# sail-sg/finetune-fair-diffusion

Measured on AMD Instinct MI355X. Metric: training-images/sec (SD-v1.5 512^2, 20-step DPM-Solver++ unroll, fairness-finetune step), higher is better.
Workload: dtype f16

## Files before the change

finetune_fair_diffusion_amd/csrc/gemm.hip:

```cpp
#include "gemm_device.h"

template <int BM, int BN, bool CONV>
__global__ __launch_bounds__(256) void gemm_glds_kernel(fd_gemm_desc p, int ntm, int ntn) {
    FD_WG_TRACE(1);
    constexpr int TM = BM / 32, TN = BN / 32;
    constexpr int AI = BM / 64, BI = BN / 64;
    constexpr int EPI_HALFS = 4 * (BM / 2) * (BN / 2 + 4);
    constexpr int OPS_HALFS = 2 * (BM + BN) * 32;
    __shared__ __attribute__((aligned(16))) f16 smem[OPS_HALFS > EPI_HALFS ? OPS_HALFS : EPI_HALFS];
    f16* As = smem;
    f16* Bs = smem + 2 * BM * 32;
    const f16* zp = fd_zero_page;
    asm volatile("" : "+s"(zp));

    const int tid = threadIdx.x, lane = tid & 63, wave = tid >> 6;
    const int l15 = lane & 15, lg = lane >> 4;
    const int wm = wave >> 1, wn = wave & 1;

    const int tile = xcd_remap(blockIdx.x, ntm * ntn);
    const int m0 = (tile / ntn) * BM, n0 = (tile % ntn) * BN;
    const int z = blockIdx.y;

    const f16* A = (const f16*)p.A + (int64_t)z * p.sA;
    const f16* B = (const f16*)p.B + (int64_t)z * p.sB;
// ... 278 lines not shown
            const bool kok = kk < Kseg;
#pragma unroll
            for (int i = 0; i < AI; ++i) {
                const int g = wave + i * NW;
                if (g < NA && (part & 1)) {
                    const int m = m0 + g * 8 + lrow;
                    const f16* src = (kok && m < p.M) ? Ap + (int64_t)m * la + kk : zp;
                    glds16(src, As + (buf * BM + g * 8) * 64);
                }
            }
#pragma unroll
            for (int i = 0; i < BI; ++i) {
                const int g = wave + i * NW;
                if (g < NB && (part & 2)) {
                    const int n = n0 + g * 8 + lrow;
                    const f16* src = (kok && n < p.N) ? Bp + (int64_t)n * lb + kk : zp;
                    glds16(src, Bs + (buf * BN + g * 8) * 64);
                }
            }
        }
    };

    f32x4 acc[TM][TN];
#pragma unroll
    for (int i = 0; i < TM; ++i)
#pragma unroll
        for (int j = 0; j < TN; ++j) acc[i][j] = (f32x4){0.f, 0.f, 0.f, 0.f};

    const int frow = l15 * 64;
    const int fsw = l15 & 7;
    const uint32_t lds0 = (uint32_t)(uintptr_t)(__attribute__((address_space(3))) void*)smem;
    constexpr bool PINNED = NW == 8;
#ifndef FD_PD
#define FD_PD 2
#endif

    const int nsplit = gridDim.y;
    const int kbeg = (int)((int64_t)nk * blockIdx.y / nsplit), kend = (int)((int64_t)nk * (blockIdx.y + 1) / nsplit);
    issue(kbeg, 0, 3);
    for (int kt = kbeg; kt < (FD_DBG_GE(p, 4) ? kbeg : kend); ++kt) {
        const int buf = (kt - kbeg) & 1;
        asm volatile("s_waitcnt vmcnt(0)" ::: "memory");
        __syncthreads();
        if (kt + 1 < kend && !FD_DBG_IS(p, 1)) issue(kt + 1, buf ^ 1, 3);
        if (FD_DBG_IS(p, 2)) continue;
        if constexpr (PINNED) {
            const uint32_t a_base = lds0 + (uint32_t)((buf * BM + wm * WTM) * 64 + frow) * 2;
            const uint32_t b_base = lds0 + (uint32_t)((2 * BM + buf * BN + wn * WTN) * 64 + frow) * 2;
#pragma unroll
            for (int ks = 0; ks < 2; ++ks) {
                const uint32_t slot = (uint32_t)(((ks * 4 + lg) ^ fsw) * 16);
                mma_k32<TM, TN, FD_PD>(acc, a_base + slot, b_base + slot);
            }
        } else {
            const f16* Ab = As + (buf * BM + wm * WTM) * 64 + frow;
            const f16* Bb = Bs + (buf * BN + wn * WTN) * 64 + frow;
#pragma unroll
            for (int ks = 0; ks < 2; ++ks) {
                const int slot = ((ks * 4 + lg) ^ fsw) * 8;
                if (TN <= TM) {
                    f16x8 bf[TN];
#pragma unroll
                    for (int j = 0; j < TN; ++j) bf[j] = *(const f16x8*)(Bb + j * 16 * 64 + slot);
                    f16x8 a0 = *(const f16x8*)(Ab + slot);
                    f16x8 a1 = *(const f16x8*)(Ab + (TM > 1 ? 1 : 0) * 16 * 64 + slot);
#pragma unroll
                    for (int i = 0; i < TM; ++i) {
                        f16x8 a2 = a1;
                        if (i + 2 < TM) a2 = *(const f16x8*)(Ab + (i + 2) * 16 * 64 + slot);
#pragma unroll
                        for (int j = 0; j < TN; ++j) acc[i][j] = FD_MFMA_16x16x32(bf[j], a0, acc[i][j]);
                        __builtin_amdgcn_sched_group_barrier(0x100, 1, 0);
                        __builtin_amdgcn_sched_group_barrier(0x008, TN, 0);
                        a0 = a1;
                        a1 = a2;
                    }
                } else {
                    f16x8 af[TM];
#pragma unroll
                    for (int i = 0; i < TM; ++i) af[i] = *(const f16x8*)(Ab + i * 16 * 64 + slot);
                    f16x8 b0 = *(const f16x8*)(Bb + slot);
                    f16x8 b1 = *(const f16x8*)(Bb + (TN > 1 ? 1 : 0) * 16 * 64 + slot);
#pragma unroll
                    for (int j = 0; j < TN; ++j) {
                        f16x8 b2 = b1;
                        if (j + 2 < TN) b2 = *(const f16x8*)(Bb + (j + 2) * 16 * 64 + slot);
#pragma unroll
                        for (int i = 0; i < TM; ++i) acc[i][j] = FD_MFMA_16x16x32(b0, af[i], acc[i][j]);
                        __builtin_amdgcn_sched_group_barrier(0x100, 1, 0);
                        __builtin_amdgcn_sched_group_barrier(0x008, TM, 0);
                        b0 = b1;
                        b1 = b2;
                    }
                }
            }
        }
    }

    if (nsplit > 1) {
        float* ws = (float*)p.workspace + (int64_t)blockIdx.y * p.M * p.N;
#pragma unroll
        for (int i = 0; i < TM; ++i) {
            const int m = m0 + wm * WTM + i * 16 + l15;
            if (m >= p.M) continue;
#pragma unroll
            for (int j = 0; j < TN; ++j) {
                const int n = n0 + wn * WTN + j * 16 + lg * 4;
                if (n < p.N) *(f32x4*)(ws + (int64_t)m * p.N + n) = acc[i][j];
            }
        }
        return;
    }
    const bool lds_epi = FD_GEMM_LDS_EPILOGUE_OK(p);
    if (FD_DBG_IS(p, 3)) {
        if (acc[0][0][0] == 12345.678f) ((f16*)p.C)[0] = (f16)1.f;
    } else if (p.act == FD_ACT_GEGLU) {
        constexpr int LDS_HALFS = 2 * (BM + BN) * 64;
        constexpr int TMC = (NW * WTM * (WTN + 4) <= LDS_HALFS) ? TM : TM / 2;
        __syncthreads();
        gemm_epilogue_geglu_lds<TM, TN, TMC>(p, acc, smem + wave * (TMC * 16) * (WTN + 4), m0 + wm * WTM, n0 + wn * WTN, lane);
    } else if (lds_epi) {
        constexpr int LDS_HALFS = 2 * (BM + BN) * 64;
        constexpr int TMC = (NW * WTM * (WTN + 4) <= LDS_HALFS) ? TM : TM / 2;
        static_assert(NW * TMC * 16 * (WTN + 4) <= LDS_HALFS, "epilogue staging does not fit");
        __syncthreads();
        gemm_epilogue_lds<TM, TN, TMC, WSTATS>(p, acc, smem + wave * (TMC * 16) * (WTN + 4), m0 + wm * WTM, n0 + wn * WTN, lane, 0, 0, up_phase);
    } else {
        gemm_epilogue<TM, TN>(p, acc, m0 + wm * WTM, n0 + wn * WTN, l15, lg, 0, 0, up_phase);
    }
}

__global__ void splitk_reduce_kernel(fd_gemm_desc p, int nsplit) {
    FD_WG_TRACE(3);
    const int64_t n4 = (int64_t)p.M * p.N / 4;
    const float* ws = (const float*)p.workspace;
    const f16* R = (const f16*)p.residual;
    const f16* RB = (const f16*)p.rowbias;
    for (int64_t i = blockIdx.x * (int64_t)blockDim.x + threadIdx.x; i < n4; i += (int64_t)gridDim.x * blockDim.x) {
        const int64_t e = i * 4;
        const int m = (int)(e / p.N), n = (int)(e - (int64_t)m * p.N);
        f32x4 a = *(const f32x4*)(ws + e);
        for (int s = 1; s < nsplit; ++s) a += *(const f32x4*)(ws + (int64_t)s * p.M * p.N + e);
        const int rbrow = RB ? m / p.rows_per_batch : 0;
        float v[4];
        const float al = n < p.colscale_cols ? p.alpha * p.colscale : p.alpha;
#pragma unroll
        for (int r = 0; r < 4; ++r) {
            float x = a[r] * al;
            if (p.bias) x += p.bias[n + r];
            if (RB) x += (float)RB[(int64_t)rbrow * p.ld_rowbias + n + r];
            x = apply_act(x, p.act);
            if (R) x += (float)R[(int64_t)m * p.ldr + n + r];
            v[r] = x;
        }
        if (p.out_dtype == FD_OUT_F32) *(f32x4*)((float*)p.C + (int64_t)m * p.ldc + n) = (f32x4){v[0], v[1], v[2], v[3]};
        else *(f16x4*)((f16*)p.C + (int64_t)m * p.ldc + n) = (f16x4){(f16)v[0], (f16)v[1], (f16)v[2], (f16)v[3]};
    }
}

static int launch_splitk_reduce(const fd_gemm_desc& d, hipStream_t s, int nsplit) {
    int64_t blocks = ((int64_t)d.M * d.N / 4 + 255) / 256;
    if (blocks > 2048) blocks = 2048;
    hipLaunchKernelGGL(splitk_reduce_kernel, dim3((unsigned)blocks), dim3(256), 0, s, d, nsplit);
    return fd_check_launch("fd_gemm(split-K reduce)");
}

template <auto KERNEL, int NTHREADS, size_t LDS>
static void launch_big_cv(const fd_gemm_desc& d, hipStream_t s, dim3 grid, int ntm, int ntn, int gn) {
    fd_allow_lds<KERNEL>(LDS);
    hipLaunchKernelGGL(KERNEL, grid, dim3(NTHREADS), LDS, s, d, ntm, ntn, gn);
}

template <int BM, int BN, int WGM, int WGN>
static int launch_big(const fd_gemm_desc& d, hipStream_t s, int nsplit, int cv) {
    const int ntm = (d.M + BM - 1) / BM, ntn = (d.N + BN - 1) / BN;
    constexpr size_t lds = (size_t)2 * (BM + BN) * 64 * sizeof(f16);
    constexpr int nt = WGM * WGN * 64;
    static const long l2_budget = bench_env("FD_GEMM_L2_KB") ? atol(bench_env("FD_GEMM_L2_KB")) * 1024 : GEMM_L2_BUDGET;
    const int gn = gemm_band_ntiles(l2_budget, BN, ((long)d.K + d.K2) / nsplit, ntn);
    const int nph = (d.conv && (d.conv_mode == FD_CONV_UP2P || d.conv_mode == FD_CONV_UP2PI)) ? 4 : 1;
    const dim3 grid(ntm * ntn * nph, nsplit);
    if (cv == 0) launch_big_cv<gemm_big_kernel<BM, BN, WGM, WGN, 0>, nt, lds>(d, s, grid, ntm, ntn, gn);
    else if (cv == 1) launch_big_cv<gemm_big_kernel<BM, BN, WGM, WGN, 1>, nt, lds>(d, s, grid, ntm, ntn, gn);
    else if (cv == 2) launch_big_cv<gemm_big_kernel<BM, BN, WGM, WGN, 2>, nt, lds>(d, s, grid, ntm, ntn, gn);
    else if constexpr (BN / WGN == 80) {
        if (cv == 6) launch_big_cv<gemm_big_kernel<BM, BN, WGM, WGN, 6>, nt, lds>(d, s, grid, ntm, ntn, gn);
        else if (cv == 3) launch_big_cv<gemm_big_kernel<BM, BN, WGM, WGN, 3>, nt, lds>(d, s, grid, ntm, ntn, gn);
        else launch_big_cv<gemm_big_kernel<BM, BN, WGM, WGN, 4>, nt, lds>(d, s, grid, ntm, ntn, gn);
    }
    if (nsplit > 1) return launch_splitk_reduce(d, s, nsplit);
    return fd_check_launch(cv >= 3 ? "fd_gemm(big, statistics epilogue)" : "fd_gemm(big)");
}


template <int NT, int KS, int RT>
__global__ __launch_bounds__(KS * 64) void gemm_skinny_kernel(fd_gemm_desc p) {
    FD_WG_TRACE(4);
    __shared__ float red[KS > 1 ? (KS - 1) * RT * NT * 256 : 1];
    const int lane = threadIdx.x & 63, wave = threadIdx.x >> 6;
    const int l15 = lane & 15, lg = lane >> 4;
    const f16* A[RT];
    bool mok[RT];
#pragma unroll
    for (int r = 0; r < RT; ++r) {
        const int m = (blockIdx.x * RT + r) * 16 + l15;
        mok[r] = m < p.M;
        A[r] = (const f16*)p.A + (int64_t)(mok[r] ? m : 0) * p.lda + lg * 8;
    }
    const f16* B = (const f16*)p.B + lg * 8;
    f32x4 acc[RT][NT];
#pragma unroll
    for (int r = 0; r < RT; ++r)
#pragma unroll
        for (int j = 0; j < NT; ++j) acc[r][j] = (f32x4){0.f, 0.f, 0.f, 0.f};
    const int nks = p.K >> 5;
    const int per = (nks + KS - 1) / KS;
    const int kbeg = wave * per, kend = min(nks, kbeg + per);
    constexpr int CH = 10 / RT;
    for (int k0 = kbeg; k0 < kend; k0 += CH) {
        f16x8 af[RT][CH];
#pragma unroll
        for (int c = 0; c < CH; ++c)
#pragma unroll
            for (int r = 0; r < RT; ++r) {
                af[r][c] = (f16x8){0, 0, 0, 0, 0, 0, 0, 0};
                if (k0 + c < kend && mok[r]) af[r][c] = *(const f16x8*)(A[r] + (int64_t)(k0 + c) * 32);
            }
#pragma unroll
        for (int c = 0; c < CH; ++c) {
            if (k0 + c < kend) {
#pragma unroll
                for (int j = 0; j < NT; ++j) {
                    const int n = j * 16 + l15;
                    f16x8 bf = (f16x8){0, 0, 0, 0, 0, 0, 0, 0};
                    if (n < p.N) bf = *(const f16x8*)(B + (int64_t)n * p.ldb + (int64_t)(k0 + c) * 32);
#pragma unroll
                    for (int r = 0; r < RT; ++r) acc[r][j] = FD_MFMA_16x16x32(bf, af[r][c], acc[r][j]);
                }
            }
        }
    }
    if (KS > 1) {
        if (wave > 0) {
#pragma unroll
            for (int r = 0; r < RT; ++r)
#pragma unroll
                for (int j = 0; j < NT; ++j) *(f32x4*)(red + ((((wave - 1) * RT + r) * NT + j) * 64 + lane) * 4) = acc[r][j];
        }
        __syncthreads();
        if (wave > 0) return;
#pragma unroll
        for (int w = 1; w < KS; ++w)
#pragma unroll
            for (int r = 0; r < RT; ++r)
#pragma unroll
                for (int j = 0; j < NT; ++j) acc[r][j] += *(const f32x4*)(red + ((((w - 1) * RT + r) * NT + j) * 64 + lane) * 4);
    }
#pragma unroll
    for (int r = 0; r < RT; ++r) {
        if (!mok[r]) continue;
        f16* C = (f16*)p.C + (int64_t)((blockIdx.x * RT + r) * 16 + l15) * p.ldc;
#pragma unroll
        for (int j = 0; j < NT; ++j) {
            const int n = j * 16 + lg * 4;
            if (n < p.N) *(f16x4*)(C + n) = (f16x4){(f16)acc[r][j][0], (f16)acc[r][j][1], (f16)acc[r][j][2], (f16)acc[r][j][3]};
        }
    }
}

static bool skinny_ok(const fd_gemm_desc& d) {
    static const bool off = bench_env("FD_GEMM_NOSKINNY") != nullptr;
    if (d.N > 16 && d.M >= 32768) return false;
    return !off && !d.conv && d.batch <= 1 && d.K2 == 0 && d.colscale_cols == 0 && d.N <= 64 && (d.N & 3) == 0 && (d.K & 31) == 0 && d.M >= 1024 && !d.bias && !d.rowbias &&
           !d.residual && d.act == FD_ACT_NONE && d.alpha == 1.f && d.out_dtype == FD_OUT_F16 && (d.ldc & 3) == 0;
}

template <int NT, int RT>
static int launch_skinny_rt(const fd_gemm_desc& d, hipStream_t s) {
    const int blocks = (d.M + 16 * RT - 1) / (16 * RT);
    const int ks = d.K >= 1280 ? 4 : d.K >= 640 ? 2 : 1;
    if (ks == 4) hipLaunchKernelGGL((gemm_skinny_kernel<NT, 4, RT>), dim3(blocks), dim3(256), 0, s, d);
    else if (ks == 2) hipLaunchKernelGGL((gemm_skinny_kernel<NT, 2, RT>), dim3(blocks), dim3(128), 0, s, d);
    else hipLaunchKernelGGL((gemm_skinny_kernel<NT, 1, RT>), dim3(blocks), dim3(64), 0, s, d);
    return fd_check_launch("fd_gemm(skinny)");
}

template <int NT>
static int launch_skinny(const fd_gemm_desc& d, hipStream_t s) {
    static const int rt = bench_env("FD_GEMM_SKINNY_RT") ? atoi(bench_env("FD_GEMM_SKINNY_RT")) : 0;
    const bool two = rt == 2;
    return two ? launch_skinny_rt<NT, 2>(d, s) : launch_skinny_rt<NT, 1>(d, s);
}

template <int BM, int BN>
static int launch(const fd_gemm_desc& d, hipStream_t s) {
    const int ntm = (d.M + BM - 1) / BM, ntn = (d.N + BN - 1) / BN;
    dim3 grid(ntm * ntn, d.batch > 0 ? d.batch : 1);
    if (d.conv) hipLaunchKernelGGL((gemm_glds_kernel<BM, BN, true>), grid, dim3(256), 0, s, d, ntm, ntn);
    else hipLaunchKernelGGL((gemm_glds_kernel<BM, BN, false>), grid, dim3(256), 0, s, d, ntm, ntn);
    return fd_check_launch("fd_gemm");
}

bool fd_gemm_pp_eligible(const fd_gemm_desc& d);
int fd_gemm_launch_pp(const fd_gemm_desc& d, hipStream_t s, bool prio, int bm, int nsplit);
bool fd_conv_halo_takes(const fd_gemm_desc& d, int bm, int nsplit);
#ifndef FD_GEMM_PP_DEFAULT
#define FD_GEMM_PP_DEFAULT (1 | 4 | 8 | 32)
#endif
static int pp_mode() {
#ifdef FD_BENCH_HOOKS
    const char* e = getenv("FD_GEMM_PP");
    return e ? atoi(e) : FD_GEMM_PP_DEFAULT;
#else
    return FD_GEMM_PP_DEFAULT;
#endif
}
static int pp_takes(const fd_gemm_desc& d, int sel) {
    const int t = sel % 1000000, split = sel / 1000000, m = pp_mode();
    if (!m || !fd_gemm_pp_eligible(d)) return 0;
    if (t == 256320 && split == 0) {
        if (d.conv) return (m & 1) ? 256 : 0;
        if ((m & 2) || ((m & 32) && d.K + d.K2 <= 384 && d.N >= 2560)) return 256;
        return 0;
    }
    if (t == 128320 && (split == 0 || (m & 64))) return (m & (d.conv ? 8 : 16)) ? 128 : 0;
    return 0;
}

static int gemm_tile(const fd_gemm_desc& d);
extern "C" int fd_gemm_tile(const fd_gemm_desc* dp) {
    FD_REQUIRE_DESC(dp, fd_gemm_desc, "fd_gemm_tile");
    return gemm_tile(*dp);
}
static int gemm_tile(const fd_gemm_desc& d) {
    const long nb = d.batch > 1 ? d.batch : 1;
    static const bool nobig = bench_env("FD_GEMM_NOBIG") != nullptr;
    static const int force = bench_env("FD_GEMM_FORCE") ? atoi(bench_env("FD_GEMM_FORCE")) : 0;
    if (skinny_ok(d)) return 16000 + (d.N + 15) / 16 * 16;
    if (force && nb == 1 && !d.conv) return force;
    static const int bigk = bench_env("FD_GEMM_BIGK") ? atoi(bench_env("FD_GEMM_BIGK")) : 320;
    if (!nobig && nb == 1 && (d.conv ? (d.Cin & 63) == 0 : (d.K + d.K2) >= bigk)) {
        const long phs = (d.conv && (d.conv_mode == FD_CONV_UP2P || d.conv_mode == FD_CONV_UP2PI)) ? 4 : 1;
        const long m256 = phs * ((d.M + 255) / 256), m128 = phs * ((d.M + 127) / 128);
        static const long t256 = bench_env("FD_GEMM_T256") ? atol(bench_env("FD_GEMM_T256")) : 100;
        static const long t128 = bench_env("FD_GEMM_T128") ? atol(bench_env("FD_GEMM_T128")) : 80;
        static const long maxsplit = bench_env("FD_GEMM_MAXSPLIT") ? atol(bench_env("FD_GEMM_MAXSPLIT")) : 8;
        static const long tc256 = bench_env("FD_CONV_T256") ? atol(bench_env("FD_CONV_T256")) : 0;
        if (d.N % 320 == 0) {
            if (m256 * (d.N / 320) >= ((tc256 && d.conv && d.conv_mode == FD_CONV_NORMAL) ? tc256 : t256)) return 256320;
            if (m128 * (d.N / 320) >= t128) return 128320;
        }
        const bool can_split = d.workspace && (d.N & 3) == 0 && (d.ldc & 3) == 0 && d.act != FD_ACT_GEGLU && phs == 1;
        const long nk = (d.K + 63) / 64 + (d.K2 + 63) / 64;
        auto split_for = [&](long blocks, int tilecode) -> int {
            long split = blocks > 0 ? 256 / blocks : 1;
            if (split > maxsplit) split = maxsplit;
            while (split > 1 && (nk / split < 8 || (int64_t)split * d.M * d.N * 4 > d.workspace_bytes)) --split;
            return split > 1 ? (int)(split * 1000000 + tilecode) : 0;
        };
        if (can_split && nk >= 64 && d.N % 320 == 0 && m128 * (d.N / 320) >= 32) {
            const int c = split_for(m128 * (d.N / 320), 128320);
            if (c) return c;
        }
        static const long t160 = bench_env("FD_GEMM_T160") ? atol(bench_env("FD_GEMM_T160")) : 160;
        if (d.N % 160 == 0 && m128 * (d.N / 160) >= t160) return 128160;
        static const bool no256 = bench_env("FD_GEMM_NO256256") != nullptr;
        static const long tvae = bench_env("FD_GEMM_TVAE") ? atol(bench_env("FD_GEMM_TVAE")) : 200;
        if (!no256 && d.N % 256 == 0 && m256 * (d.N / 256) >= tvae) return 256256;
        static const bool no512 = bench_env("FD_GEMM_NO512128") != nullptr;
        if (!no512 && d.N == 128 && ((d.M + 511) / 512) >= 400) return 512128;
        if (d.N % 128 == 0 && m256 * (d.N / 128) >= tvae) return 256128;
        if (can_split && d.N % 160 == 0) {
            const int c = split_for(m128 * (d.N / 160), 128160);
            if (c) return c;
        }
    }
    const long t128 = (long)((d.M + 127) / 128) * ((d.N + 127) / 128) * nb;
    const bool n64 = (d.N % 128) != 0 && (d.N % 128) <= 64;
    if (t128 >= 512 && !n64) return 128128;
    const long t12864 = (long)((d.M + 127) / 128) * ((d.N + 63) / 64) * nb;
    if (t12864 >= 512) return 128064;
    return 64064;
}

enum { GK_SKINNY, GK_GLDS, GK_BIG, GK_PP };
struct GemmPlan {
    int kind, bm, bn, wgm, wgn, nsplit, cv;
    bool stats_ok;
    int big_cv(bool st) const { return st ? (cv == 2 ? 6 : cv + 3) : cv; }
};
static fd_gemm_desc normalise_k2(fd_gemm_desc d) {
    if (d.K2 <= 0 || !d.A2) d.K2 = 0;
    return d;
}
static GemmPlan gemm_plan(const fd_gemm_desc& d ) {
    GemmPlan g = {};
    const int sel = gemm_tile(d), t = sel % 1000000;
    static const bool w16 = bench_env("FD_GEMM_W8") == nullptr;
    g.nsplit = sel >= 1000000 ? sel / 1000000 : 1;
    g.bm = t / 1000; g.bn = t % 1000;
    g.cv = d.conv ? (d.conv_mode >= FD_CONV_UP2P ? 2 : 1) : 0;
    if (const int bm = pp_takes(d, sel)) { g.kind = GK_PP; g.bm = bm; g.bn = 320; g.wgm = 2; g.wgn = 4; }
    else if (g.nsplit > 1) { g.kind = GK_BIG; g.wgm = 4; g.wgn = t == 128320 ? 4 : 2; }
    else switch (t) {
        case 256320: g.kind = GK_BIG; g.wgm = (w16 && !d.conv) ? 4 : 2; g.wgn = 4; break;
        case 128320: g.kind = GK_BIG; g.wgm = w16 ? 4 : 2; g.wgn = 4; break;
        case 128160: g.kind = GK_BIG; g.wgm = 4; g.wgn = 2; break;
        case 256256: g.kind = GK_BIG; g.wgm = 2; g.wgn = 4; break;
        case 512128: g.kind = GK_BIG; g.wgm = 8; g.wgn = 2; break;
        case 256128: g.kind = GK_BIG; g.wgm = 4; g.wgn = 2; break;
        default: g.kind = g.bm == 16 ? GK_SKINNY : GK_GLDS; break;
    }
    g.stats_ok = (g.kind == GK_PP || (g.kind == GK_BIG && g.bn / g.wgn == 80)) && g.nsplit == 1 && FD_GEMM_LDS_EPILOGUE_OK(d) && d.act != FD_ACT_GEGLU &&
                 d.batch <= 1 && (d.N % 80) == 0 && (g.cv < 2 || (d.conv_mode == FD_CONV_UP2PI && (d.M & 31) == 0));
    return g;
}

extern "C" int fd_gemm_kernel_name(const fd_gemm_desc* dp, char* buf, int n) {
    FD_REQUIRE_DESC(dp, fd_gemm_desc, "fd_gemm_kernel_name");
    const fd_gemm_desc d = normalise_k2(*dp);
    const GemmPlan g = gemm_plan(d);
    const bool st = d.gn_stats && g.stats_ok;
    switch (g.kind) {
        case GK_PP:
            if (fd_conv_halo_takes(d, g.bm, g.nsplit)) snprintf(buf, n, "conv_halo_kernel<%d, %d, %d, true>", g.bm, d.W, st ? 3 : 1);
            else snprintf(buf, n, "gemm_pp_kernel<%d, %d, %s>", g.bm, (d.conv ? 1 : 0) + (st ? 2 : 0), (pp_mode() & 4) ? "true" : "false");
            break;
        case GK_BIG: snprintf(buf, n, "gemm_big_kernel<%d, %d, %d, %d, %d>", g.bm, g.bn, g.wgm, g.wgn, g.big_cv(st)); break;
        case GK_SKINNY: snprintf(buf, n, "gemm_skinny_kernel<%d, %d, 1>", g.bn / 16, d.K >= 1280 ? 4 : d.K >= 640 ? 2 : 1); break;
        default: snprintf(buf, n, "gemm_glds_kernel<%d, %d, %s>", g.bm, g.bn, d.conv ? "true" : "false"); break;
    }
    return g.nsplit > 1 ? g.nsplit : 0;
}

extern "C" int fd_gemm_stats_rows(const fd_gemm_desc* dp) {
    FD_REQUIRE_DESC(dp, fd_gemm_desc, "fd_gemm_stats_rows");
    return gemm_plan(normalise_k2(*dp)).stats_ok ? 32 : 0;
}

extern "C" int fd_gemm(const fd_gemm_desc* dp, void* stream) {
    FD_REQUIRE_DESC(dp, fd_gemm_desc, "fd_gemm");
    fd_gemm_desc d = *dp;
#ifdef FD_BENCH_HOOKS
    static const char* dbg = bench_env("FD_GEMM_DBG");
    if (dbg && d.batch <= 1) d.batch = -atoi(dbg);
#endif
    FD_REQUIRE(d.A && d.B && d.C, "fd_gemm: null operand");
    FD_REQUIRE(d.M > 0 && d.N > 0 && d.K > 0, "fd_gemm: bad shape M=%d N=%d K=%d", d.M, d.N, d.K);
    FD_REQUIRE((d.K & 7) == 0 && (d.lda & 7) == 0 && (d.ldb & 7) == 0, "fd_gemm: K, lda, ldb must be multiples of 8");
    if (d.K2 > 0) {
        FD_REQUIRE(!d.conv, "fd_gemm: second K-slab not supported with conv gather");
        FD_REQUIRE(d.A2 && d.B2 && (d.K2 & 7) == 0 && (d.lda2 & 7) == 0 && (d.ldb2 & 7) == 0, "fd_gemm: bad second slab");
        FD_REQUIRE(d.batch <= 1, "fd_gemm: second slab is not batched");
    }
    d = normalise_k2(d);
    if (d.conv) {
        const bool up_fwd = d.conv_mode == FD_CONV_UP2P || d.conv_mode == FD_CONV_UP2PI;
        const int ntap = up_fwd ? 4 : d.conv_mode == FD_CONV_UP2P_BWD ? 16 : 9;
        FD_REQUIRE((d.Cin & 31) == 0 && d.K == ntap * d.Cin, "fd_gemm(conv): Cin must be a multiple of 32 and K == taps*Cin");
        if (up_fwd) FD_REQUIRE(!d.residual && !d.rowbias, "fd_gemm(conv up2 phases): bias-only epilogue");
        if (d.conv_mode == FD_CONV_UP2PI) FD_REQUIRE(d.out_dtype == FD_OUT_F16, "fd_gemm(conv up2 phases, interleaved result): fp16 output");
        FD_REQUIRE(d.M == d.Bn * d.Ho * d.Wo, "fd_gemm(conv): M != B*Ho*Wo");
        FD_REQUIRE(d.batch <= 1, "fd_gemm(conv): not batched");
        FD_REQUIRE((int64_t)d.Bn * d.H * d.W * d.lda < (1LL << 31), "fd_gemm(conv): input larger than 2^31 elements");
    }
    if (d.rowbias) FD_REQUIRE(d.rows_per_batch > 0, "fd_gemm: rows_per_batch");
    FD_REQUIRE(d.colscale_cols >= 0 && (d.colscale_cols & 3) == 0 && (d.colscale_cols == 0 || (d.act != FD_ACT_GEGLU && d.batch <= 1)),
               "fd_gemm: colscale_cols=%d must be a multiple of 4 (not with GEGLU / batched launches)", d.colscale_cols);
    if (d.act == FD_ACT_GEGLU)
        FD_REQUIRE(!d.conv && d.batch <= 1 && d.out_dtype == FD_OUT_F16 && !d.rowbias && d.alpha == 1.f && (d.N & 15) == 0 &&
                       (d.ldc & 7) == 0 && d.K2 == 0 && (!d.residual || (d.ldr & 7) == 0),
                   "fd_gemm(GEGLU): needs a plain fp16 GEMM with N %% 16 == 0 and ldc, ldr %% 8 == 0");
    hipStream_t s = (hipStream_t)stream;
    const GemmPlan g = gemm_plan(d);
    if (d.gn_stats) FD_REQUIRE(g.stats_ok, "fd_gemm: gn_stats set but the kernel for M=%d N=%d K=%d has no statistics epilogue (ask fd_gemm_stats_rows first)",
                               d.M, d.N, d.K);
    if (d.conv && d.conv_mode >= FD_CONV_UP2P)
        FD_REQUIRE(g.kind == GK_BIG, "fd_gemm(conv up2 phases): shape not taken by the big-tile kernels (Cin %% 64, enough tiles); use FD_CONV_UP2");
    switch (g.kind) {
        case GK_PP: {
            const int rc = fd_gemm_launch_pp(d, s, (pp_mode() & 4) != 0, g.bm, g.nsplit);
            if (rc != 0 || g.nsplit == 1) return rc;
            return launch_splitk_reduce(d, s, g.nsplit);
        }
        case GK_SKINNY:
            switch (g.bn) {
                case 16: return launch_skinny<1>(d, s);
                case 32: return launch_skinny<2>(d, s);
                case 48: return launch_skinny<3>(d, s);
                default: return launch_skinny<4>(d, s);
            }
        case GK_BIG: {
            const int cv = g.big_cv(d.gn_stats != nullptr);
            switch (g.bm * 1000 + g.bn) {
                case 256320: return g.wgm == 4 ? launch_big<256, 320, 4, 4>(d, s, g.nsplit, cv) : launch_big<256, 320, 2, 4>(d, s, g.nsplit, cv);
                case 128320: return g.wgm == 4 ? launch_big<128, 320, 4, 4>(d, s, g.nsplit, cv) : launch_big<128, 320, 2, 4>(d, s, g.nsplit, cv);
                case 128160: return launch_big<128, 160, 4, 2>(d, s, g.nsplit, cv);
                case 256256: return launch_big<256, 256, 2, 4>(d, s, g.nsplit, cv);
                case 512128: return launch_big<512, 128, 8, 2>(d, s, g.nsplit, cv);
                default: return launch_big<256, 128, 4, 2>(d, s, g.nsplit, cv);
            }
        }
        default:
            if (g.bm == 128 && g.bn == 128) return launch<128, 128>(d, s);
            if (g.bm == 128 && g.bn == 64) return launch<128, 64>(d, s);
            return launch<64, 64>(d, s);
    }
}

FD_WGT_SETTER(gemm)
```

finetune_fair_diffusion_amd/csrc/gemm_pp.hip:

```cpp
#include "gemm_pp_device.h"

constexpr uint32_t PP_OOR = 0xFFFFFFF0u;
template <int BM, int CV, bool PRIO>
__global__ __launch_bounds__(512) void gemm_pp_kernel(fd_gemm_desc p, int ntm, int ntn, int gn) {
    FD_WG_TRACE(5);
    constexpr int CONV = CV & 1;
    constexpr bool WSTATS = CV >= 2;
    constexpr int WTM = BM / 2, WTN = 80, TM = WTM / 16, TN = 5;
    constexpr int NGA = BM / 16, NAW = NGA / PP_NW;
    constexpr int STAGE = pp_stage<BM>();
    extern __shared__ __attribute__((aligned(16))) f16 smem[];
    const f16* zp = fd_zero_page;
    asm volatile("" : "+s"(zp));

    const int tid = threadIdx.x, lane = tid & 63;
    const int wave = __builtin_amdgcn_readfirstlane(tid >> 6);
    const int l15 = lane & 15, lg = lane >> 4;
    const int wm = wave >> 2, wn = wave & 3;
    const bool lead = wave < 4;

    int tile = xcd_remap(blockIdx.x, gridDim.x);
    int mt, nt;
    if (gn >= ntn) {
        mt = tile / ntn;
        nt = tile - mt * ntn;
    } else {
        const int per = ntm * gn, nbands = (ntn + gn - 1) / gn;
        const int band = min(tile / per, nbands - 1);
        const int r = tile - band * per;
        const int w = band == nbands - 1 ? ntn - band * gn : gn;
        mt = r / w;
        nt = band * gn + (r - mt * w);
    }
    const int m0 = mt * BM, n0 = nt * PP_BN;

    const f16* A = (const f16*)p.A;
    const f16* B = (const f16*)p.B;
    const int nk1 = (p.K + 31) >> 5, nk2 = (p.K2 + 31) >> 5, nkt = nk1 + nk2;
    const int nsplit = gridDim.y;
    const int kbeg = (int)((int64_t)nkt * blockIdx.y / nsplit), kend = (int)((int64_t)nkt * (blockIdx.y + 1) / nsplit);
    const int nk = kend - kbeg;

    const int lrow = lane >> 2;
    const int kchunk = ((lane & 3) ^ swz_g(lane >> 4)) * 8;
    int a_off[NAW], a_mask[NAW];
#pragma unroll
    for (int i = 0; i < NAW; ++i) {
        const int m = m0 + (wave + 8 * i) * 16 + lrow;
        const bool valid = m < p.M;
        if (CONV) {
            const int hw = p.Ho * p.Wo;
            const int mm = valid ? m : 0;
            const int b = mm / hw;
            const int r = mm - b * hw;
            const int oy = r / p.Wo;
            const int ox = r - oy * p.Wo;
            int mask = 0;
#pragma unroll
            for (int t = 0; t < 9; ++t) {
                const int iy = oy + t / 3 - 1, ix = ox + t % 3 - 1;
                if (valid && iy >= 0 && iy < p.H && ix >= 0 && ix < p.W) mask |= 1 << t;
            }
            a_off[i] = (int)(((int64_t)(b * p.H + oy) * p.W + ox) * p.lda) + kchunk;
            a_mask[i] = mask;
        } else {
            a_off[i] = valid ? m : -1;
            a_mask[i] = 0;
        }
    }
    int b_row[3];
#pragma unroll
    for (int i = 0; i < 3; ++i) {
        const int n = n0 + (wave + 8 * i) * 16 + lrow;
        b_row[i] = (n < p.N && (wave + 8 * i) < PP_NGB) ? n : -1;
    }
    f16* const dump = smem + PP_NST * STAGE + wave * PP_GROUP;
#if __HIP_DEVICE_COMPILE__
    __amdgpu_buffer_rsrc_t rA, rB, rA2, rB2;
    uint32_t a_vo[NAW], a_vo2[NAW], b_vo[3], b_vo2[3];
    if (!CONV) {
        auto rsrc = [](const void* base, int64_t rows, int64_t ld, int k) {
            const int64_t bytes = base ? ((rows - 1) * ld + k) * 2 : 0;
            return __builtin_amdgcn_make_buffer_rsrc((void*)base, 0, (int)(uint32_t)bytes, 0x00020000);
        };
        rA = rsrc(p.A, p.M, p.lda, p.K); rB = rsrc(p.B, p.N, p.ldb, p.K);
        rA2 = rsrc(p.K2 ? p.A2 : nullptr, p.M, p.lda2, p.K2); rB2 = rsrc(p.K2 ? p.B2 : nullptr, p.N, p.ldb2, p.K2);
#pragma unroll
        for (int i = 0; i < NAW; ++i) {
            a_vo[i] = a_off[i] >= 0 ? (uint32_t)(a_off[i] * (int)p.lda + kchunk) * 2 : PP_OOR;
            a_vo2[i] = a_off[i] >= 0 ? (uint32_t)(a_off[i] * (int)p.lda2 + kchunk) * 2 : PP_OOR;
        }
#pragma unroll
        for (int i = 0; i < 3; ++i) {
            b_vo[i] = b_row[i] >= 0 ? (uint32_t)(b_row[i] * (int)p.ldb + kchunk) * 2 : PP_OOR;
            b_vo2[i] = b_row[i] >= 0 ? (uint32_t)(b_row[i] * (int)p.ldb2 + kchunk) * 2 : PP_OOR;
        }
    }
#endif

    auto issue = [&](int j, auto nl_c) {
        constexpr int NL = decltype(nl_c)::value;
        if (j >= nk || (FD_DBG_IS(p, 1) && j >= 3)) {
#pragma unroll
            for (int i = 0; i < NL; ++i) glds16(zp, dump);
            return;
        }
        const int kt = kbeg + j;
        f16* st = smem + (j & 3) * STAGE;
        if (CONV) {
            const int cc = kt / 9;
            const int tap = kt - cc * 9;
            const int c0 = cc << 5;
            const int ky = tap / 3, kx = tap - ky * 3;
            const int toff = ((ky - 1) * p.W + (kx - 1)) * (int)p.lda + c0;
#pragma unroll
            for (int i = 0; i < NAW; ++i) {
                const f16* src = ((a_mask[i] >> tap) & 1) ? A + (int64_t)(a_off[i] + toff) : zp;
                glds16(src, st + (wave + 8 * i) * PP_GROUP);
            }
            const int kk = tap * p.Cin + c0 + kchunk;
#pragma unroll
            for (int i = 0; i < NL - NAW; ++i) {
                const f16* src = b_row[i] >= 0 ? B + (int64_t)b_row[i] * p.ldb + kk : zp;
                glds16(src, st + (NGA + wave + 8 * i) * PP_GROUP);
            }
        } else {
#if __HIP_DEVICE_COMPILE__
            const bool seg2 = kt >= nk1;
            const int k0 = (seg2 ? kt - nk1 : kt) * 32;
            const int rem = (seg2 ? p.K2 : p.K) - k0;
            const bool kok = kchunk < rem;
            const uint32_t so = (uint32_t)k0 * 2;
            if (!seg2) {
#pragma unroll
                for (int i = 0; i < NAW; ++i)
                    __builtin_amdgcn_raw_ptr_buffer_load_lds(rA, (__attribute__((address_space(3))) void*)(st + (wave + 8 * i) * PP_GROUP), 16, kok ? a_vo[i] : PP_OOR, so, 0, 0);
#pragma unroll
                for (int i = 0; i < NL - NAW; ++i)
                    __builtin_amdgcn_raw_ptr_buffer_load_lds(rB, (__attribute__((address_space(3))) void*)(st + (NGA + wave + 8 * i) * PP_GROUP), 16, kok ? b_vo[i] : PP_OOR, so, 0, 0);
            } else {
#pragma unroll
                for (int i = 0; i < NAW; ++i)
                    __builtin_amdgcn_raw_ptr_buffer_load_lds(rA2, (__attribute__((address_space(3))) void*)(st + (wave + 8 * i) * PP_GROUP), 16, kok ? a_vo2[i] : PP_OOR, so, 0, 0);
#pragma unroll
                for (int i = 0; i < NL - NAW; ++i)
                    __builtin_amdgcn_raw_ptr_buffer_load_lds(rB2, (__attribute__((address_space(3))) void*)(st + (NGA + wave + 8 * i) * PP_GROUP), 16, kok ? b_vo2[i] : PP_OOR, so, 0, 0);
            }
#endif
        }
    };

    f32x4 acc[TM][TN];
#pragma unroll
    for (int i = 0; i < TM; ++i)
#pragma unroll
        for (int j = 0; j < TN; ++j) acc[i][j] = (f32x4){0.f, 0.f, 0.f, 0.f};

    const uint32_t lds0 = (uint32_t)(uintptr_t)(__attribute__((address_space(3))) void*)smem;
    const uint32_t frag = (uint32_t)(l15 * 32 + ((lg ^ swz_g(l15 >> 2)) * 8)) * 2;
    const uint32_t a_frag = lds0 + (uint32_t)(wm * (WTM / 16) * PP_GROUP) * 2 + frag;
    const uint32_t b_frag = lds0 + (uint32_t)((NGA + wn * (WTN / 16)) * PP_GROUP) * 2 + frag;
    constexpr uint32_t STAGE_B = STAGE * 2, GROUP_B = PP_GROUP * 2;

    auto main_loop = [&](auto abl_c, auto nosync_c) {
        constexpr int ABL = decltype(abl_c)::value;
        constexpr bool NOSYNC = decltype(nosync_c)::value;
        if (lead) {
            constexpr int NL = NAW + 3;
            std::integral_constant<int, NL> nl;
            issue(0, nl); issue(1, nl); issue(2, nl);
            wait_vm<2 * NL>();
            raw_barrier();
            for (int i = 0; i < nk; ++i) {
                const uint32_t so = (uint32_t)(i & 3) * STAGE_B;
                auto mid = [&] {
                    if (!NOSYNC) {
                        wait_vm<NL>();
                        raw_barrier();
                    }
                };
                mma_k32_mid<TM, TN, 2, GROUP_B, PRIO, decltype(mid)&, ABL>(acc, a_frag + so, b_frag + so, mid);
                issue(i + 3, nl);
            }
        } else {
            constexpr int NL = NAW + 2;
            std::integral_constant<int, NL> nl;
            issue(0, nl); issue(1, nl); issue(2, nl);
            wait_vm<2 * NL>();
            raw_barrier();
            for (int i = 0; i < nk; ++i) {
                if (!NOSYNC) {
                    wait_vm<NL>();
                    raw_barrier();
                }
                issue(i + 3, nl);
                const uint32_t so = (uint32_t)(i & 3) * STAGE_B;
                auto mid = [] {};
                mma_k32_mid<TM, TN, 2, GROUP_B, PRIO, decltype(mid)&, ABL>(acc, a_frag + so, b_frag + so, mid);
            }
        }
    };
#ifdef FD_BENCH_HOOKS
    if (FD_DBG_IS(p, 2)) main_loop(std::integral_constant<int, 2>{}, std::false_type{});
    else if (FD_DBG_IS(p, 6)) main_loop(std::integral_constant<int, 6>{}, std::false_type{});
    else if (FD_DBG_IS(p, 7)) main_loop(std::integral_constant<int, 0>{}, std::true_type{});
    else
#endif
    main_loop(std::integral_constant<int, 0>{}, std::false_type{});
    if (nsplit > 1) {
        float* ws = (float*)p.workspace + (int64_t)blockIdx.y * p.M * p.N;
#pragma unroll
        for (int i = 0; i < TM; ++i) {
            const int m = m0 + wm * WTM + i * 16 + l15;
            if (m >= p.M) continue;
#pragma unroll
            for (int j = 0; j < TN; ++j) {
                const int n = n0 + wn * WTN + j * 16 + lg * 4;
                if (n < p.N) *(f32x4*)(ws + (int64_t)m * p.N + n) = acc[i][j];
            }
        }
        return;
    }
    asm volatile("s_waitcnt vmcnt(0)" ::: "memory");
    __syncthreads();
    if (FD_DBG_IS(p, 3)) {
        if (acc[0][0][0] == 12345.678f) ((f16*)p.C)[0] = (f16)1.f;
        return;
    }

    const bool lds_epi = FD_GEMM_LDS_EPILOGUE_OK(p);
    constexpr int TMC = BM == 256 ? TM / 2 : TM;
    static_assert(PP_NW * TMC * 16 * (WTN + 4) <= PP_NST * STAGE, "epilogue staging does not fit the ring");
    if (p.act == FD_ACT_GEGLU) {
        gemm_epilogue_geglu_lds<TM, TN, TMC>(p, acc, smem + wave * (TMC * 16) * (WTN + 4), m0 + wm * WTM, n0 + wn * WTN, lane);
    } else if (lds_epi) {
        gemm_epilogue_lds<TM, TN, TMC, WSTATS>(p, acc, smem + wave * (TMC * 16) * (WTN + 4), m0 + wm * WTM, n0 + wn * WTN, lane, 0, 0);
    } else {
        gemm_epilogue<TM, TN>(p, acc, m0 + wm * WTM, n0 + wn * WTN, l15, lg, 0, 0);
    }
}

template <int BM, int CV, bool PRIO>
static void launch_pp(const fd_gemm_desc& d, hipStream_t s, int ntm, int ntn, int gn, int nsplit) {
    fd_allow_lds<gemm_pp_kernel<BM, CV, PRIO>>(pp_lds<BM>());
    hipLaunchKernelGGL((gemm_pp_kernel<BM, CV, PRIO>), dim3(ntm * ntn, nsplit), dim3(512), pp_lds<BM>(), s, d, ntm, ntn, gn);
}

template <int BM>
static void launch_pp_bm(const fd_gemm_desc& d, hipStream_t s, bool prio, int nsplit) {
    const int ntm = (d.M + BM - 1) / BM, ntn = d.N / PP_BN;
    const int gn = gemm_band_ntiles(GEMM_L2_BUDGET, PP_BN, ((long)d.K + d.K2) / nsplit, ntn);
    if (d.gn_stats && nsplit == 1) {
        if (d.conv) { if (prio) launch_pp<BM, 3, true>(d, s, ntm, ntn, gn, 1); else launch_pp<BM, 3, false>(d, s, ntm, ntn, gn, 1); }
        else { if (prio) launch_pp<BM, 2, true>(d, s, ntm, ntn, gn, 1); else launch_pp<BM, 2, false>(d, s, ntm, ntn, gn, 1); }
        return;
    }
    if (d.conv) { if (prio) launch_pp<BM, 1, true>(d, s, ntm, ntn, gn, nsplit); else launch_pp<BM, 1, false>(d, s, ntm, ntn, gn, nsplit); }
    else { if (prio) launch_pp<BM, 0, true>(d, s, ntm, ntn, gn, nsplit); else launch_pp<BM, 0, false>(d, s, ntm, ntn, gn, nsplit); }
}

bool fd_gemm_pp_eligible(const fd_gemm_desc& d) {
    if (d.batch > 1 || (d.N % 320) != 0) return false;
    if (d.conv) return d.conv_mode == FD_CONV_NORMAL && (d.Cin & 31) == 0 && d.K2 == 0;
    const int64_t lim = 1LL << 31;
    return (d.K & 7) == 0 && (int64_t)d.M * d.lda < lim && (int64_t)d.N * d.ldb < lim && (d.K2 == 0 || ((int64_t)d.M * d.lda2 < lim && (int64_t)d.N * d.ldb2 < lim));
}

bool fd_conv_halo_eligible(const fd_gemm_desc& d, int bm);
int fd_conv_halo_launch(const fd_gemm_desc& d, hipStream_t s, int bm);
bool fd_conv_halo_takes(const fd_gemm_desc& d, int bm, int nsplit) {
#ifdef FD_BENCH_HOOKS
    const char* e = getenv("FD_CONV_HALO");
    if (e && atoi(e) == 0) return false;
#endif
    return nsplit == 1 && fd_conv_halo_eligible(d, bm);
}

int fd_gemm_launch_pp(const fd_gemm_desc& d, hipStream_t s, bool prio, int bm, int nsplit) {
    if (fd_conv_halo_takes(d, bm, nsplit)) return fd_conv_halo_launch(d, s, bm);
    if (bm == 256) launch_pp_bm<256>(d, s, prio, nsplit);
    else launch_pp_bm<128>(d, s, prio, nsplit);
    return fd_check_launch("fd_gemm(pp)");
}

FD_WGT_SETTER(gemm_pp)
```

Measured before the change: 6.165.

## Walk multiple N tiles per workgroup in pp GEMM to read A once

Adds a row-walk mode to the ping-pong GEMM kernel for non-conv, small-K shapes: each workgroup loops over several consecutive N tiles of the same M row block instead of one tile. The goal is to fetch each A row block from HBM roughly once and keep the B panel L2-resident, cutting DRAM traffic on memory-bound tall-skinny GEMMs. The walk width is the largest value that still leaves at least 256 workgroups. The trade-off is fewer workgroups and serialised tiles per workgroup, with an extra barrier between tiles, which can lower occupancy and latency hiding. Also adds profiling scratch scripts.

```diff
diff --git a/finetune_fair_diffusion_amd/csrc/gemm.hip b/finetune_fair_diffusion_amd/csrc/gemm.hip
--- a/finetune_fair_diffusion_amd/csrc/gemm.hip
+++ b/finetune_fair_diffusion_amd/csrc/gemm.hip
@@ -604,7 +604,7 @@
 }
 
 bool fd_gemm_pp_eligible(const fd_gemm_desc& d);
-int fd_gemm_launch_pp(const fd_gemm_desc& d, hipStream_t s, bool prio, int bm, int nsplit);
+int fd_gemm_launch_pp(const fd_gemm_desc& d, hipStream_t s, bool prio, int bm, int nsplit, int walk);
 bool fd_conv_halo_takes(const fd_gemm_desc& d, int bm, int nsplit);
 #ifndef FD_GEMM_PP_DEFAULT
 #define FD_GEMM_PP_DEFAULT (1 | 4 | 8 | 32)
@@ -688,6 +688,7 @@
 enum { GK_SKINNY, GK_GLDS, GK_BIG, GK_PP };
 struct GemmPlan {
     int kind, bm, bn, wgm, wgn, nsplit, cv;
+    int walk;
     bool stats_ok;
     int big_cv(bool st) const { return st ? (cv == 2 ? 6 : cv + 3) : cv; }
 };
@@ -695,6 +696,18 @@
     if (d.K2 <= 0 || !d.A2) d.K2 = 0;
     return d;
 }
+constexpr long GEMM_WALK_MIN_WGS = 256;
+static int gemm_row_walk(const fd_gemm_desc& d, int bm, int bn, int nsplit) {
+    static const bool off = bench_env("FD_GEMM_NOWALK") != nullptr;
+    if (off || d.conv || d.gn_stats || nsplit > 1 || d.batch > 1) return 1;
+    const long ktot = (long)d.K + d.K2;
+    const long ntm = (d.M + bm - 1) / bm, ntn = (d.N + bn - 1) / bn;
+    if (ktot > 640 || ntn < 2 || ntn * bn * ktot * 2 > GEMM_L2_BUDGET) return 1;
+    for (long w = ntn; w > 1; --w)
+        if (ntm * ((ntn + w - 1) / w) >= GEMM_WALK_MIN_WGS) return (int)w;
+    return 1;
+}
+
 static GemmPlan gemm_plan(const fd_gemm_desc& d ) {
     GemmPlan g = {};
     const int sel = gemm_tile(d), t = sel % 1000000;
@@ -713,6 +726,7 @@
         case 256128: g.kind = GK_BIG; g.wgm = 4; g.wgn = 2; break;
         default: g.kind = g.bm == 16 ? GK_SKINNY : GK_GLDS; break;
     }
+    g.walk = g.kind == GK_PP ? gemm_row_walk(d, g.bm, g.bn, g.nsplit) : 1;
     g.stats_ok = (g.kind == GK_PP || (g.kind == GK_BIG && g.bn / g.wgn == 80)) && g.nsplit == 1 && FD_GEMM_LDS_EPILOGUE_OK(d) && d.act != FD_ACT_GEGLU &&
                  d.batch <= 1 && (d.N % 80) == 0 && (g.cv < 2 || (d.conv_mode == FD_CONV_UP2PI && (d.M & 31) == 0));
     return g;
@@ -738,6 +752,11 @@
 extern "C" int fd_gemm_stats_rows(const fd_gemm_desc* dp) {
     FD_REQUIRE_DESC(dp, fd_gemm_desc, "fd_gemm_stats_rows");
     return gemm_plan(normalise_k2(*dp)).stats_ok ? 32 : 0;
+}
+
+extern "C" int fd_gemm_row_walk(const fd_gemm_desc* dp) {
+    FD_REQUIRE_DESC(dp, fd_gemm_desc, "fd_gemm_row_walk");
+    return gemm_plan(normalise_k2(*dp)).walk;
 }
 
 extern "C" int fd_gemm(const fd_gemm_desc* dp, void* stream) {
@@ -781,7 +800,7 @@
         FD_REQUIRE(g.kind == GK_BIG, "fd_gemm(conv up2 phases): shape not taken by the big-tile kernels (Cin %% 64, enough tiles); use FD_CONV_UP2");
     switch (g.kind) {
         case GK_PP: {
-            const int rc = fd_gemm_launch_pp(d, s, (pp_mode() & 4) != 0, g.bm, g.nsplit);
+            const int rc = fd_gemm_launch_pp(d, s, (pp_mode() & 4) != 0, g.bm, g.nsplit, g.walk);
             if (rc != 0 || g.nsplit == 1) return rc;
             return launch_splitk_reduce(d, s, g.nsplit);
         }
diff --git a/finetune_fair_diffusion_amd/csrc/gemm_pp.hip b/finetune_fair_diffusion_amd/csrc/gemm_pp.hip
--- a/finetune_fair_diffusion_amd/csrc/gemm_pp.hip
+++ b/finetune_fair_diffusion_amd/csrc/gemm_pp.hip
@@ -13,12 +13,6 @@
     const f16* zp = fd_zero_page;
     asm volatile("" : "+s"(zp));
 
-    const int tid = threadIdx.x, lane = tid & 63;
-    const int wave = __builtin_amdgcn_readfirstlane(tid >> 6);
-    const int l15 = lane & 15, lg = lane >> 4;
-    const int wm = wave >> 2, wn = wave & 3;
-    const bool lead = wave < 4;
-
     int tile = xcd_remap(blockIdx.x, gridDim.x);
     int mt, nt;
     if (gn >= ntn) {
@@ -32,7 +26,28 @@
         mt = r / w;
         nt = band * gn + (r - mt * w);
     }
-    const int m0 = mt * BM, n0 = nt * PP_BN;
+    int nwalk = 1;
+    if constexpr (CV == 0) {
+        if (gn < 0) {
+            const int groups = (ntn - gn - 1) / -gn;
+            mt = tile / groups;
+            nt = (tile - mt * groups) * -gn;
+            nwalk = min(-gn, ntn - nt);
+        }
+    }
+    int n0 = nt * PP_BN;
+
+    for (int walk = 0;; ++walk) {
+    int tid = threadIdx.x, m0 = mt * BM;
+    if constexpr (CV == 0) {
+        asm volatile("" : "+v"(tid));
+        asm volatile("" : "+s"(m0));
+    }
+    const int lane = tid & 63;
+    const int wave = __builtin_amdgcn_readfirstlane(tid >> 6);
+    const int l15 = lane & 15, lg = lane >> 4;
+    const int wm = wave >> 2, wn = wave & 3;
+    const bool lead = wave < 4;
 
     const f16* A = (const f16*)p.A;
     const f16* B = (const f16*)p.B;
@@ -238,18 +253,26 @@
     } else {
         gemm_epilogue<TM, TN>(p, acc, m0 + wm * WTM, n0 + wn * WTN, l15, lg, 0, 0);
     }
+    if constexpr (CV != 0) break;
+    else {
+        if (walk + 1 >= nwalk) break;
+        n0 += PP_BN;
+        __syncthreads();
+    }
+    }
 }
 
 template <int BM, int CV, bool PRIO>
 static void launch_pp(const fd_gemm_desc& d, hipStream_t s, int ntm, int ntn, int gn, int nsplit) {
     fd_allow_lds<gemm_pp_kernel<BM, CV, PRIO>>(pp_lds<BM>());
-    hipLaunchKernelGGL((gemm_pp_kernel<BM, CV, PRIO>), dim3(ntm * ntn, nsplit), dim3(512), pp_lds<BM>(), s, d, ntm, ntn, gn);
+    const int nwg = gn < 0 ? ntm * ((ntn - gn - 1) / -gn) : ntm * ntn;
+    hipLaunchKernelGGL((gemm_pp_kernel<BM, CV, PRIO>), dim3(nwg, nsplit), dim3(512), pp_lds<BM>(), s, d, ntm, ntn, gn);
 }
 
 template <int BM>
-static void launch_pp_bm(const fd_gemm_desc& d, hipStream_t s, bool prio, int nsplit) {
+static void launch_pp_bm(const fd_gemm_desc& d, hipStream_t s, bool prio, int nsplit, int walk) {
     const int ntm = (d.M + BM - 1) / BM, ntn = d.N / PP_BN;
-    const int gn = gemm_band_ntiles(GEMM_L2_BUDGET, PP_BN, ((long)d.K + d.K2) / nsplit, ntn);
+    const int gn = walk > 1 ? -walk : gemm_band_ntiles(GEMM_L2_BUDGET, PP_BN, ((long)d.K + d.K2) / nsplit, ntn);
     if (d.gn_stats && nsplit == 1) {
         if (d.conv) { if (prio) launch_pp<BM, 3, true>(d, s, ntm, ntn, gn, 1); else launch_pp<BM, 3, false>(d, s, ntm, ntn, gn, 1); }
         else { if (prio) launch_pp<BM, 2, true>(d, s, ntm, ntn, gn, 1); else launch_pp<BM, 2, false>(d, s, ntm, ntn, gn, 1); }
@@ -276,10 +299,10 @@
     return nsplit == 1 && fd_conv_halo_eligible(d, bm);
 }
 
-int fd_gemm_launch_pp(const fd_gemm_desc& d, hipStream_t s, bool prio, int bm, int nsplit) {
+int fd_gemm_launch_pp(const fd_gemm_desc& d, hipStream_t s, bool prio, int bm, int nsplit, int walk) {
     if (fd_conv_halo_takes(d, bm, nsplit)) return fd_conv_halo_launch(d, s, bm);
-    if (bm == 256) launch_pp_bm<256>(d, s, prio, nsplit);
-    else launch_pp_bm<128>(d, s, prio, nsplit);
+    if (bm == 256) launch_pp_bm<256>(d, s, prio, nsplit, walk);
+    else launch_pp_bm<128>(d, s, prio, nsplit, walk);
     return fd_check_launch("fd_gemm(pp)");
 }
 
diff --git a/scratch/a_once_summary.py b/scratch/a_once_summary.py
--- /dev/null
+++ b/scratch/a_once_summary.py
@@ -0,0 +1,58 @@
+import csv, glob, json, os, re, statistics, sys, collections
+ROOT = os.path.dirname(os.path.dirname(os.path.abspath(__file__)))
+OUT = os.environ.get("FD_PROF_OUT") or os.path.join(ROOT, "prof_out")
+SHAPES = [(65536, 320, 320, "none"), (65536, 960, 320, "none"), (65536, 1280, 320, "none"), (65536, 2560, 320, "geglu"),
+          (16384, 1920, 640, "none"), (16384, 2560, 640, "none"), (16384, 320, 640, "none")]
+NP = 6
+tag, tdir, fdir, wdir = sys.argv[1:5]
+GEMM = re.compile(r"gemm_(big|pp|glds)_kernel")
+
+
+def files(d, suffix):
+    return glob.glob(os.path.join(d, "**", "*" + suffix), recursive=True)
+
+
+def trace(d):
+    rows = []
+    for f in files(d, "kernel_trace.csv"):
+        for r in csv.DictReader(open(f)):
+            if GEMM.search(r["Kernel_Name"]):
+                rows.append((int(r["Start_Timestamp"]), (int(r["End_Timestamp"]) - int(r["Start_Timestamp"])) / 1e3, r["Kernel_Name"],
+                             int(r.get("Grid_Size_X", r.get("Grid_Size", 0)) or 0) // max(int(r.get("Workgroup_Size_X", r.get("Workgroup_Size", 1)) or 1), 1)))
+    rows.sort()
+    return rows
+
+
+def counter(d, name):
+    per = collections.OrderedDict()
+    rows = []
+    for f in files(d, "counter_collection.csv"):
+        for r in csv.DictReader(open(f)):
+            if GEMM.search(r["Kernel_Name"]) and r["Counter_Name"] == name:
+                rows.append((int(r["Dispatch_Id"]), float(r["Counter_Value"])))
+    rows.sort()
+    for i, v in rows:
+        per[i] = per.get(i, 0.0) + v
+    return list(per.values())
+
+
+T, F, W = trace(tdir), counter(fdir, "FETCH_SIZE"), counter(wdir, "WRITE_SIZE")
+print("dispatches: trace %d fetch %d write %d (expected %d)" % (len(T), len(F), len(W), NP * len(SHAPES)))
+out = []
+for s, (M, N, K, act) in enumerate(SHAPES):
+    t = T[s * NP:(s + 1) * NP]
+    us = [x[1] for x in t[2:]]
+    f = [2.0 * v * 1024 / 1e6 for v in F[s * NP + 2:(s + 1) * NP]]
+    w = [v * 1024 / 1e6 for v in W[s * NP + 2:(s + 1) * NP]]
+    out_mb = M * (N // 2 + N if act == "geglu" else N) * 2 / 1e6
+    ab_mb = (M * K + N * K) * 2 / 1e6
+    row = dict(M=M, N=N, K=K, act=act, kernel=t[-1][2] if t else "?", workgroups=t[-1][3] if t else 0,
+               us_median=round(statistics.median(us), 2) if us else None, us_all=[round(x, 1) for x in us],
+               read_mb=round(statistics.mean(f), 1) if f else None, write_mb=round(statistics.mean(w), 1) if w else None,
+               a_plus_b_mb=round(ab_mb, 1), out_mb=round(out_mb, 1))
+    if us:
+        row["us_per_out_mb"] = round(row["us_median"] / out_mb, 4)
+        row["tb_s_on_needed_bytes"] = round((ab_mb + out_mb) / row["us_median"], 3)
+    out.append(row)
+    print(json.dumps(row))
+json.dump(out, open(os.path.join(OUT, "a_once", "pmc_%s.json" % tag), "w"), indent=1)
diff --git a/scratch/mb_a_once.py b/scratch/mb_a_once.py
--- /dev/null
+++ b/scratch/mb_a_once.py
@@ -0,0 +1,79 @@
+import json, os, statistics, sys
+ROOT = os.path.dirname(os.path.dirname(os.path.abspath(__file__)))
+OUT = os.environ.get("FD_PROF_OUT") or os.path.join(ROOT, "prof_out")
+sys.path.insert(0, ROOT)
+import torch
+from finetune_fair_diffusion_amd import ops, lib
+
+SHAPES = [(65536, 320, 320, "none"), (65536, 960, 320, "none"), (65536, 1280, 320, "none"), (65536, 2560, 320, "geglu"),
+          (16384, 1920, 640, "none"), (16384, 2560, 640, "none"), (16384, 320, 640, "none")]
+NP = 6
+dev = torch.device("cuda")
+
+
+def setup(M, N, K, act):
+    nb = int(700e6 // (M * K * 2)) + 1
+    g = torch.Generator(device=dev).manual_seed(1)
+    xs = [torch.randn(M, K, device=dev, generator=g).half() for _ in range(nb)]
+    w = (torch.randn(N, K, device=dev, generator=g) * 0.02).half()
+    bias = torch.randn(N, device=dev, generator=g)
+    no = 3
+    if act == "geglu":
+        outs = [torch.empty(M, N // 2, device=dev, dtype=torch.float16) for _ in range(no)]
+        auxs = [torch.empty(M, N, device=dev, dtype=torch.float16) for _ in range(no)]
+    else:
+        outs = [torch.empty(M, N, device=dev, dtype=torch.float16) for _ in range(no)]
+        auxs = [None] * no
+
+    def run(i, hot=False):
+        ops.gemm(xs[0 if hot else i % nb], w, bias=bias, act=act, out=outs[i % no], aux=auxs[i % no])
+    return run
+
+
+def kname(M, N, K, act):
+    import ctypes
+    d = lib.GemmDesc()
+    d.M, d.N, d.K, d.lda, d.ldb, d.ldc, d.batch, d.act = M, N, K, K, K, N, 1, ops.ACT[act]
+    d.A = d.B = d.C = 1
+    buf = ctypes.create_string_buffer(128)
+    lib.get().fd_gemm_kernel_name(ctypes.byref(d), buf, 128)
+    return buf.value.decode()
+
+
+mode = sys.argv[1]
+os.makedirs(os.path.join(OUT, "a_once"), exist_ok=True)
+if mode == "pmc":
+    for (M, N, K, act) in SHAPES:
+        run = setup(M, N, K, act)
+        for i in range(NP):
+            run(i)
+        torch.cuda.synchronize()
+        del run
+        torch.cuda.empty_cache()
+    print("pmc done")
+else:
+    tag = sys.argv[2]
+    res = []
+    for (M, N, K, act) in SHAPES:
+        run = setup(M, N, K, act)
+        row = dict(M=M, N=N, K=K, act=act, kernel=kname(M, N, K, act))
+        for hot in (False, True):
+            for i in range(4):
+                run(i, hot)
+            ts = []
+            for i in range(15):
+                a, b = torch.cuda.Event(enable_timing=True), torch.cuda.Event(enable_timing=True)
+                a.record(); run(i + 4, hot); b.record()
+                ts.append((a, b))
+            torch.cuda.synchronize()
+            us = sorted(1e3 * a.elapsed_time(b) for a, b in ts)
+            row["hot_us" if hot else "cold_us"] = dict(median=round(statistics.median(us), 2), min=round(us[0], 2), max=round(us[-1], 2))
+        out_mb = M * (N // 2 + N if act == "geglu" else N) * 2 / 1e6
+        need_mb = (M * K + N * K) * 2 / 1e6 + out_mb
+        row.update(out_mb=round(out_mb, 1), need_mb=round(need_mb, 1), us_per_out_mb=round(row["cold_us"]["median"] / out_mb, 4),
+                   tb_s_needed=round(need_mb / row["cold_us"]["median"], 3))
+        res.append(row)
+        print(json.dumps(row), flush=True)
+        del run
+        torch.cuda.empty_cache()
+    json.dump(res, open(os.path.join(OUT, "a_once", "time_%s.json" % tag), "w"), indent=1)
```

Result: no change. 6.130 (-0.6%).
